# rlvc/FEALESS

Hardware: AMD Instinct MI355X
Metric: frames/sec (640x480 RGB-D x N templates, 20 ICP iters) (higher is better)
Workload: dtype u8

## Files before the change

fealess_amd/_lib.py:

```python
import ctypes as C
import os

_HERE = os.path.dirname(os.path.abspath(__file__))
LIB_PATH = os.environ.get("FEALESS_HIP_LIB") or os.path.join(_HERE, "csrc", "libfealess_hip.so")

FL_OK = 0
FL_ERR_INVALID, FL_ERR_HIP, FL_ERR_ASSERT, FL_ERR_OVERFLOW, FL_ERR_NO_DEVICE, FL_ERR_STATE, FL_ERR_NO_TEMPLATE = -1, -2, -3, -4, -5, -6, -7
FL_MEM_HOST, FL_MEM_DEVICE = 0, 1
FL_ICP_PARITY, FL_ICP_FAST, FL_ICP_POINT_TO_PLANE = 0, 1, 2


class Feature(C.Structure):
    _fields_ = [("x", C.c_int32), ("y", C.c_int32), ("label", C.c_int32)]


class Template(C.Structure):
    _fields_ = [("width", C.c_int32), ("height", C.c_int32), ("offset_x", C.c_int32), ("offset_y", C.c_int32),
                ("pyramid_level", C.c_int32), ("feat_begin", C.c_int32), ("feat_count", C.c_int32)]


class Match(C.Structure):
    _fields_ = [("x", C.c_int32), ("y", C.c_int32), ("similarity", C.c_float), ("class_idx", C.c_int32),
                ("template_id", C.c_int32)]

# ... 133 lines not shown
    "fl_recognize_topk": (_I, [_P, _P, _P, _I, C.POINTER(Intrinsics), C.POINTER(RecognitionParams), _I, _P, C.POINTER(_I)]),
    "fl_recognize_batch_topk": (_I, [_P, _I, C.POINTER(_P), C.POINTER(_P), _I, C.POINTER(Intrinsics), C.POINTER(RecognitionParams), _I, _P,
                                     C.POINTER(_I)]),
    "fl_group_matches": (_I, [_P, _P, _I, _I, C.POINTER(InstanceParams), _P, _P, _P]),
    "fl_recognize_batch_instances": (_I, [_P, _I, C.POINTER(_P), C.POINTER(_P), _I, C.POINTER(Intrinsics), C.POINTER(RecognitionParams),
                                          C.POINTER(InstanceParams), _P, C.POINTER(C.c_int32), C.POINTER(C.c_int32)]),
    "fl_tracker_create": (_I, [_P, _P, _I, _P, _I, _I, _I, _I, _I, _I, C.POINTER(_P)]),
    "fl_tracker_destroy": (None, [_P]),
    "fl_track_batch": (_I, [_P, _I, C.POINTER(_P), _I, _I, _P, _P, C.POINTER(Intrinsics), C.POINTER(TrackParams), _P]),
    "fl_verify_batch": (_I, [_P, _I, C.POINTER(_P), _I, _I, _P, _P, _I, _P, C.POINTER(Intrinsics), C.POINTER(VerifyParams), _P]),
    "fl_nms": (_I, [_P, _I, _F, C.POINTER(_I), C.POINTER(_I)]),
    "fl_export_topk": (_I, [_P, _I, _I, _I, _P]),
    "fl_merge_topk": (_I, [_P, _I, _P, _I]),
    "fl_export_topk_batch": (_I, [_P, _I, _I, _I, _P]),
    "fl_merge_topk_batch": (_I, [_P, _I, _I, _I, _P, _I, C.POINTER(_I)]),
    "fl_refine_matches": (_I, [_P, _I, C.POINTER(C.c_int32), _P, C.POINTER(Intrinsics), C.POINTER(RecognitionParams), _P]),
    "fl_select_best_batch": (_I, [_P, _P, _I, _I, _I, _I, _I, _P]),
    "fl_refine_selected": (_I, [_P, _I, C.POINTER(Intrinsics), C.POINTER(RecognitionParams), _P, C.c_size_t, _P]),
    "fl_last_stage_times": (_I, [_P, C.POINTER(StageTimes)]),
    "fl_frame_counters": (_I, [_P, _I, C.POINTER(C.c_int32)]),
}

DEV_SIGNATURES = {
    "fl_dev_detector_create_host": (_I, [_I, _I, C.POINTER(_I), C.POINTER(_P)]),
    "fl_dev_group_jobs": (_I, [_P, _P, _I, C.POINTER(InstanceParams), _P, _P, _P, _P, _P]),
    "fl_dev_extract_select": (_I, [_P, _I, _P]),
    "fl_dev_front_images": (_I, [_P, _P, _P, _I, _I, _I, _I, _P, C.c_size_t]),
    "fl_dev_tracker_create_host": (_I, [_I, _I, _I, _I, _I, C.POINTER(_P)]),
    "fl_dev_tracker_stage_ms": (_I, [_P, C.POINTER(C.c_float)]),
    "fl_dev_tracker_verify_ms": (_I, [_P, C.POINTER(C.c_float)]),
    "fl_dev_cq_window_addr": (None, [C.c_uint, _I, _I, C.POINTER(C.c_uint), C.POINTER(C.c_uint), C.POINTER(_I)]),
    "fl_dev_cq_window_taps": (None, [_P, C.c_uint, _I, _I, _I, _I, _P]),
    "fl_dev_scan_items": (_I, [_P, _I, _I, _I, C.c_uint, _P, _I, _P, _I, _P]),
}


def dev(lib, name):
    fn = getattr(lib, name)
    fn.restype, fn.argtypes = DEV_SIGNATURES[name]
    return fn


class MgResult(C.Structure):
    _fields_ = [("status", C.c_int32), ("found", C.c_int32), ("best", Match), ("pose", C.c_float * 16)]


FL_MG_ID_BYTES = 128
MG_LIB_PATH = os.path.join(_HERE, "mg", "libfealess_mg.so")
MG_SIGNATURES = {
    "fl_mg_unique_id": (_I, [_P, C.c_size_t]),
    "fl_mg_create": (_I, [_P, _P, _I, _I, _I, _I, _I, C.POINTER(_P)]),
    "fl_mg_destroy": (None, [_P]),
    "fl_mg_last_error": (C.c_char_p, [_P]),
    "fl_mg_recognize_batch": (_I, [_P, _I, C.POINTER(_P), C.POINTER(_P), _I, C.POINTER(Intrinsics), C.POINTER(RecognitionParams), _P]),
    "fl_mg_last_stats": (_I, [_P, C.POINTER(C.c_int32), C.POINTER(C.c_size_t), C.POINTER(C.c_size_t)]),
}

_lib = None
_mg_lib = None


def load_mg():
    global _mg_lib
    if _mg_lib is None:
        load()
        if not os.path.exists(MG_LIB_PATH):
# ... 26 lines not shown
```

fealess_amd/csrc/fl_context.hip:

```cpp
#include "fl_internal.h"
#include <stdlib.h>
#include <stdarg.h>
#include <string.h>
#include <algorithm>

int fl_set_error(fl_context *ctx, int code, const char *fmt, ...)
{
  if (ctx) {
    va_list ap;
    va_start(ap, fmt);
    vsnprintf(ctx->err, sizeof(ctx->err), fmt, ap);
    va_end(ap);
  }
  return code;
}

int fl_scratch(fl_context *ctx, size_t bytes, void **out)
{
  if (int rc = fl_context_join(ctx)) return rc;
  if (bytes > ctx->scratch_bytes) {
    if (ctx->scratch) {
      FL_HIP(ctx, hipStreamSynchronize(ctx->stream));
      FL_HIP(ctx, hipFree(ctx->scratch));
      ctx->scratch = nullptr;
// ... 46 lines not shown
  const long mode = ctx->opt.pipeline_icp;
  if (ctx->icp_stream && ctx->icp_stream_mode != mode) {
    FL_HIP(ctx, hipStreamSynchronize(ctx->icp_stream));
    FL_HIP(ctx, hipStreamDestroy(ctx->icp_stream));
    ctx->icp_stream = nullptr;
  }
  if (!ctx->icp_stream) {
    int least = 0, greatest = 0;
    FL_HIP(ctx, hipDeviceGetStreamPriorityRange(&least, &greatest));
    FL_HIP(ctx, hipStreamCreateWithPriority(&ctx->icp_stream, hipStreamNonBlocking, mode == 2 ? greatest : (mode == 3 ? least : 0)));
    ctx->icp_stream_mode = mode;
  }
  if (!ctx->ev_icp_tail) FL_HIP(ctx, hipEventCreateWithFlags(&ctx->ev_icp_tail, hipEventDisableTiming));
  *out = ctx->icp_stream;
  return FL_OK;
}

extern "C" int fl_abi_version(void) { return FL_ABI_VERSION; }

struct FlOptionName { const char *name, *env; long fl_context::Options::*field; bool hex; long lo, hi; };
static const FlOptionName fl_option_names[] = {
  {"scan_prune", "FL_SCAN_PRUNE", &fl_context::Options::scan_prune, false, 0, 1},
  {"scan_prune_mid", "FL_SCAN_PRUNE_MID", &fl_context::Options::scan_prune_mid, true, -1, 0xFF},
  {"icp_wide", "FL_ICP_WIDE", &fl_context::Options::icp_wide, false, -1, 1},
  {"icp_occ", "FL_ICP_OCC", &fl_context::Options::icp_occ, false, 0, 5},
  {"icp_order", "FL_ICP_ORDER", &fl_context::Options::icp_order, false, 0, 1},
  {"icp_wg_per_cu", "FL_ICP_WG_PER_CU", &fl_context::Options::icp_wg_per_cu, false, 0, 3},
  {"eager_frontend", "FL_EAGER_FRONTEND", &fl_context::Options::eager_frontend, false, 0, 1},
  {"dev_poison", "FL_DEV_POISON", &fl_context::Options::dev_poison, false, 0, 1},
  {"ws_pad", "FL_DEV_WS_PAD", &fl_context::Options::ws_pad, false, 0, 16l << 20},
  {"pipeline_icp", "FL_PIPELINE_ICP", &fl_context::Options::pipeline_icp, false, 0, 3},
  {"frontend_chunk_rows", "FL_FRONTEND_CHUNK_ROWS", &fl_context::Options::frontend_chunk_rows, false, 0, 60 * 1024},
  {"scan_run", "FL_SCAN_RUN", &fl_context::Options::scan_run, false, 0, 64},
};

static bool fl_option_valid(const FlOptionName &o, long v)
{
  if (v < o.lo || v > o.hi) return false;
  if (o.field == &fl_context::Options::frontend_chunk_rows) return v % 60 == 0;
  return o.field != &fl_context::Options::icp_occ || v == 0 || v >= 4;
}

extern "C" int fl_context_create(int device, fl_context **out)
{
  if (!out) return FL_ERR_INVALID;
  *out = nullptr;
  int n = 0;
  if (hipGetDeviceCount(&n) != hipSuccess || n <= 0) return FL_ERR_NO_DEVICE;
  if (device < 0 || device >= n) return FL_ERR_INVALID;
  fl_context *ctx = new fl_context();
  ctx->device = device;
  if (hipSetDevice(device) != hipSuccess ||
      hipStreamCreateWithFlags(&ctx->own_stream, hipStreamNonBlocking) != hipSuccess) {
    delete ctx;
    return FL_ERR_HIP;
  }
  ctx->stream = ctx->own_stream;
  {
    hipDeviceProp_t prop;
    if (hipGetDeviceProperties(&prop, device) == hipSuccess && prop.multiProcessorCount > 0) ctx->cus = prop.multiProcessorCount;
  }
  for (const FlOptionName &o : fl_option_names)
    if (const char *e = getenv(o.env)) {
      const long v = o.hex ? (long)strtoul(e, nullptr, 16) : atol(e);
      if (fl_option_valid(o, v)) ctx->opt.*(o.field) = v;
    }
// ... 65 lines not shown
extern "C" size_t fl_lm_label_stride(int w, int h, int T)
{
  size_t W = (size_t)(w / T), H = (size_t)(h / T);
  size_t pad = W * H + 16 * W + 64;
  size_t s = (size_t)T * T * W * H + pad;
  return (s + 63) & ~(size_t)63;
}

extern "C" int fl_detector_create(fl_context *ctx, int modalities, int levels, const int *T_at_level,
                                  fl_detector **out)
{
  if (!ctx || !out || !T_at_level) return FL_ERR_INVALID;
  if (modalities < 1 || modalities > FL_MAX_MODALITIES || levels < 1 || levels > FL_MAX_LEVELS)
    return fl_set_error(ctx, FL_ERR_INVALID, "modalities must be 1..%d and levels 1..%d", FL_MAX_MODALITIES,
                        FL_MAX_LEVELS);
  for (int l = 0; l < levels; ++l)
    if (T_at_level[l] < 1 || T_at_level[l] > 16) return fl_set_error(ctx, FL_ERR_INVALID, "T out of range");
  fl_detector *det = new fl_detector();
  det->ctx = ctx;
  ++ctx->detectors;
  det->M = modalities;
  det->L = levels;
  for (int l = 0; l < levels; ++l) det->T[l] = T_at_level[l];
  memset(&det->times, 0, sizeof(det->times));
  *out = det;
  return FL_OK;
}

static void free_device_tables(fl_detector *det)
{
  (void)hipFree(det->d_scan_items);
  (void)hipFree(det->d_scan_off);
  (void)hipFree(det->d_fine_hdr);
  (void)hipFree(det->d_fine_feat);
  (void)hipFree(det->d_pyr);
  (void)hipFree(det->d_poses);
  (void)hipFree(det->d_class_first);
  (void)hipFree(det->d_item_enabled);
  (void)hipFree((void *)det->d_depth_ptrs);
  (void)hipFree(det->d_ws);
  (void)hipFree(det->d_results);
  if (det->h_results) (void)hipHostFree(det->h_results);
  det->d_scan_items = nullptr;
  det->n_scan_items = 0;
  det->scan_item_g.clear();
  det->d_scan_off = nullptr;
  det->d_fine_hdr = nullptr;
  det->d_fine_feat = nullptr;
  det->d_pyr = nullptr;
  det->d_poses = nullptr;
  det->d_class_first = nullptr;
  det->d_item_enabled = nullptr;
  det->d_depth_ptrs = nullptr;
  det->d_ws = nullptr;
  det->d_results = nullptr;
  det->h_results = nullptr;
  for (auto &e : det->ev)
    if (e) { (void)hipEventDestroy(e); e = nullptr; }
  for (int b = 0; b < 2; ++b) {
    if (det->ev_done[b]) { (void)hipEventDestroy(det->ev_done[b]); det->ev_done[b] = nullptr; }
    if (det->ev_set_read[b]) { (void)hipEventDestroy(det->ev_set_read[b]); det->ev_set_read[b] = nullptr; }
    det->set_busy[b] = false;
  }
  det->prev_n = 0;
  det->latest_open = false;
  if (det->d_jobs) { (void)hipFree(det->d_jobs); det->d_jobs = nullptr; }
  if (det->d_icp_order) { (void)hipFree(det->d_icp_order); det->d_icp_order = nullptr; }
  det->selected_frames = 0;
  if (det->d_zoom) { (void)hipFree(det->d_zoom); det->d_zoom = nullptr; }
  if (det->d_zoom_src) { (void)hipFree(det->d_zoom_src); det->d_zoom_src = nullptr; det->zoom_src_bytes = 0; }
  for (int b = 0; b < 2; ++b) {
    if (det->d_in[b]) { (void)hipFree(det->d_in[b]); det->d_in[b] = nullptr; }
    if (det->ev_up[b]) { (void)hipEventDestroy(det->ev_up[b]); det->ev_up[b] = nullptr; }
    if (det->ev_read[b]) { (void)hipEventDestroy(det->ev_read[b]); det->ev_read[b] = nullptr; }
    det->read_pending[b] = false;
  }
  if (det->copy_stream) { (void)hipStreamSynchronize(det->copy_stream); (void)hipStreamDestroy(det->copy_stream); det->copy_stream = nullptr; }
}

extern "C" void fl_detector_destroy(fl_detector *det)
// ... 267 lines not shown
  free_device_tables(det);
  det->finalized = false;
  fl_batch_forget(det);
  const int L = det->L, M = det->M;
  int cap = max_candidates > 0 ? max_candidates : (max_candidates < 0 ? -max_candidates : 65536);
  det->cap_hard = max_candidates < 0;
  int cap2 = 1;
  while (cap2 < cap) cap2 <<= 1;
  cap = cap2;

  for (int l = 0; l < L; ++l) {
    FlLevelGeom &g = det->geom[l];
    g.w = w0 >> l;
    g.h = h0 >> l;
    g.T = det->T[l];
    if (g.w <= 0 || g.h <= 0) return fl_set_error(ctx, FL_ERR_INVALID, "level %d is empty", l);
    if (g.w % g.T || g.h % g.T)
      return fl_set_error(ctx, FL_ERR_ASSERT, "level %d: %dx%d not divisible by T=%d (CV_Assert linemod.cpp:1062)", l, g.w,
                          g.h, g.T);
    if ((g.w * g.h) % 16) return fl_set_error(ctx, FL_ERR_ASSERT, "level %d: rows*cols %% 16 != 0 (linemod.cpp:981)", l);
    g.W = g.w / g.T;
    g.H = g.h / g.T;
    g.WH = g.W * g.H;
    size_t s = fl_lm_label_stride(g.w, g.h, g.T);
    if (8 * s > 0xFFFFFFFFull) return fl_set_error(ctx, FL_ERR_INVALID, "linear memory too large");
    g.stride = (uint32_t)s;
    g.zero_off = (uint32_t)(7 * s + (size_t)g.T * g.T * g.WH);
  }

  std::vector<FlScanHdr> scan_hdr;
  std::vector<uint32_t> scan_off;
  std::vector<FlFineHdr> fine_hdr;
  std::vector<FlFineFeat> fine_feat;
  std::vector<FlPyrInfo> pyr;
  std::vector<float> poses;
  std::vector<const uint16_t *> depth_ptrs;
  std::vector<int> class_first;
  int g_idx = 0;
  double scan_bytes = 0.0;
  det->max_tw = det->max_th = 1;
  det->depth_w = det->depth_h = 0;
  for (size_t ci = 0; ci < det->classes.size(); ++ci) {
    FlClass &c = det->classes[ci];
    c.first_g = g_idx;
    class_first.push_back(g_idx);
    if (c.d_depths) {
      if (c.dw != w0 || c.dh != h0)
        return fl_set_error(ctx, FL_ERR_INVALID, "model depth renders must be %dx%d like the frames", w0, h0);
      det->depth_w = c.dw;
      det->depth_h = c.dh;
    }
    for (int p = 0; p < c.n_pyramids; ++p, ++g_idx) {
      const fl_template *tp = &c.templates[(size_t)p * L * M];
      FlPyrInfo pi;
      pi.class_idx = (int)ci;
      pi.template_id = p;
      pi.off_x0 = tp[0].offset_x;
      pi.off_y0 = tp[0].offset_y;
      pi.width0 = tp[0].width;
      pi.height0 = tp[0].height;
      const bool has_depth = c.d_depths && c.has_depth[(size_t)p];
      pi.depth_slot = has_depth ? p : -1;
      pi.pad = 0;
      pyr.push_back(pi);
      det->max_tw = std::max(det->max_tw, std::min(tp[0].width, w0));
      det->max_th = std::max(det->max_th, std::min(tp[0].height, h0));
      for (int k = 0; k < 13; ++k) poses.push_back(c.poses.empty() ? 0.f : c.poses[(size_t)p * 13 + k]);
      depth_ptrs.push_back(has_depth ? c.d_depths + (size_t)p * c.dw * c.dh : nullptr);
      {
        const FlLevelGeom &g = det->geom[L - 1];
        for (int m = 0; m < M; ++m) {
          const fl_template &t = tp[(L - 1) * M + m];
          FlScanHdr h;
          int wf = (t.width - 1) / g.T + 1, hf = (t.height - 1) / g.T + 1;
          int span_x = g.W - wf, span_y = g.H - hf;
          h.P = span_y * g.W + span_x + 1;
          if (h.P > g.WH) h.P = g.WH;
          h.off_begin = (int)scan_off.size();
          h.nf = t.feat_count;
          int n = 0;
          for (int k = 0; k < t.feat_count; ++k) {
            const fl_feature &f = c.features[t.feat_begin + k];
            if (f.x < 0 || f.x >= g.w || f.y < 0 || f.y >= g.h) continue;
            uint32_t off = (uint32_t)f.label * g.stride + (uint32_t)((f.y % g.T) * g.T + (f.x % g.T)) * g.WH +
                           (uint32_t)((f.y / g.T) * g.W + f.x / g.T);
            scan_off.push_back(off);
            ++n;
          }
          while (n % 8) { scan_off.push_back(g.zero_off); ++n; }
          h.n_pad = n;
          scan_hdr.push_back(h);
          const double Pd = h.P > 0 ? (double)h.P : 0.0;
          scan_bytes += (double)t.feat_count * Pd + Pd + (m == 0 ? 2.0 * Pd : 0.0);
        }
      }
      for (int l = 0; l < L - 1; ++l) {
        for (int m = 0; m < M; ++m) {
          const fl_template &t = tp[l * M + m];
          FlFineHdr h;
          h.feat_begin = (int)fine_feat.size();
          h.feat_count = t.feat_count;
          h.width = t.width;
          h.height = t.height;
          for (int k = 0; k < t.feat_count; ++k) {
            const fl_feature &f = c.features[t.feat_begin + k];
            FlFineFeat ff;
            ff.x = (int16_t)f.x;
            ff.y = (int16_t)f.y;
            {
              const int Tl = det->geom[l].T;
              const int rx = ((f.x % Tl) + Tl) % Tl, ry = ((f.y % Tl) + Tl) % Tl;
              ff.gx = (uint8_t)rx;
              ff.gy = (uint8_t)ry;
              ff.qx = (int16_t)((f.x - rx) / Tl);
              ff.qy = (int16_t)((f.y - ry) / Tl);
              ff.label = (uint8_t)f.label;
              ff.pad = 0;
            }
            fine_feat.push_back(ff);
          }
          fine_hdr.push_back(h);
        }
      }
    }
  }
  det->n_pyr = g_idx;
  det->scan_bytes_per_frame = scan_bytes;

  int rc;
  {
    std::vector<FlScanItem> items;
    fl_build_scan_items(scan_hdr, g_idx, M, det->geom[L - 1].WH, det->geom[L - 1].zero_off, scan_off, items);
    det->n_scan_items = (int)items.size();
    det->scan_item_g.clear();
    for (const FlScanItem &it : items) det->scan_item_g.push_back(it.g);
    if ((rc = upload(ctx, items, &det->d_scan_items))) return rc;
  }
  if ((rc = upload(ctx, scan_off, &det->d_scan_off))) return rc;
  if ((rc = upload(ctx, fine_hdr, &det->d_fine_hdr))) return rc;
  if ((rc = upload(ctx, fine_feat, &det->d_fine_feat))) return rc;
  if ((rc = upload(ctx, pyr, &det->d_pyr))) return rc;
  if ((rc = upload(ctx, poses, &det->d_poses))) return rc;
  if ((rc = upload(ctx, class_first, &det->d_class_first))) return rc;
  if ((rc = fl_apply_class_filter(det))) return rc;
  {
    const uint16_t **tmp = nullptr;
    if ((rc = upload(ctx, depth_ptrs, (const uint16_t ***)&tmp))) return rc;
    det->d_depth_ptrs = tmp;
  }

  det->w0 = w0;
  det->h0 = h0;
  det->max_batch = max_batch;
  det->eager_env = ctx->opt.eager_frontend != 0;
  det->poison_env = ctx->opt.dev_poison != 0;
  if ((rc = layout_workspace(det, cap))) return rc;
  if ((rc = fl_icp_prepare(det))) return rc;
  FL_HIP(ctx, hipMalloc((void **)&det->d_results, sizeof(fl_recognition_result) * (size_t)max_batch));
  FL_HIP(ctx, hipHostMalloc((void **)&det->h_results, sizeof(fl_recognition_result) * 2 * (size_t)max_batch,
                            hipHostMallocDefault));
  for (auto &e : det->ev) FL_HIP(ctx, hipEventCreate(&e));
  for (int b = 0; b < 2; ++b) {
    FL_HIP(ctx, hipEventCreateWithFlags(&det->ev_done[b], hipEventDisableTiming));
    FL_HIP(ctx, hipEventCreateWithFlags(&det->ev_set_read[b], hipEventDisableTiming));
  }
  det->finalized = true;
  return FL_OK;
}
```

fealess_amd/csrc/fl_internal.h:

```cpp
#pragma once
#include <hip/hip_runtime.h>
#include <cmath>
#include <stdint.h>
#include <stdio.h>
#include <string>
#include <vector>
#include "../../include/fealess_hip.h"

#define FL_WAVE 64

struct fl_context {
  int device = 0;
  hipStream_t own_stream = nullptr;
  hipStream_t stream = nullptr;
  hipStream_t icp_stream = nullptr;
  long icp_stream_mode = 0;
  hipEvent_t ev_icp_tail = nullptr;
  bool icp_pending = false;
  char err[512] = {0};
  void *scratch = nullptr;
  size_t scratch_bytes = 0;
  void *pinned = nullptr;
  size_t pinned_bytes = 0;
  int cus = 256;
  struct Options {
    long scan_prune = 1;
    long scan_prune_mid = -1;
    long icp_wide = -1;
    long icp_occ = 0;
    long icp_order = 1;
    long icp_wg_per_cu = 0;
    long eager_frontend = 0;
    long dev_poison = 0;
    long ws_pad = 0;
    long pipeline_icp = 3;
    long frontend_chunk_rows = 0;
    long scan_run = 0;
  } opt;
  int detectors = 0;
  bool destroy_pending = false;
};

int fl_set_error(fl_context *ctx, int code, const char *fmt, ...);
int fl_scratch(fl_context *ctx, size_t bytes, void **out);
int fl_pinned(fl_context *ctx, size_t bytes, void **out);
int fl_context_join(fl_context *ctx);
int fl_context_sync_all(fl_context *ctx);
int fl_icp_stream(fl_context *ctx, hipStream_t *out);

#define FL_HIP(ctx, call)                                                                  \
  do {                                                                                     \
    hipError_t e_ = (call);                                                                \
    if (e_ != hipSuccess)                                                                  \
      return fl_set_error((ctx), FL_ERR_HIP, "%s:%d: %s -> %s", __FILE__, __LINE__, #call, \
                          hipGetErrorString(e_));                                          \
  } while (0)

static inline size_t fl_align(size_t v, size_t a) { return (v + a - 1) / a * a; }
static inline bool fl_finite_all(const float *p, size_t n)
{
  for (size_t i = 0; i < n; ++i)
    if (!std::isfinite(p[i])) return false;
  return true;
}

#define FL_MAX_LEVELS 4
#define FL_MAX_MODALITIES 2
#define FL_MAX_FEATURES 63

struct FlScanHdr {
  int32_t P;
  int32_t off_begin;
  int32_t n_pad;
  int32_t nf;
};
struct FlScanItem {
  uint32_t off0[8];
  int32_t g;
  uint32_t chunk_nf;
  struct {
    int32_t P;
    int32_t off_begin;
    uint32_t npad_nf;
  } mod[FL_MAX_MODALITIES];
};
static_assert(sizeof(FlScanItem) == 64 && FL_MAX_MODALITIES == 2, "a dword per lane of a 16-lane load");
#define FL_SCAN_OFF_PAD 8
void fl_build_scan_items(const std::vector<FlScanHdr> &hdr, int n_pyr, int M, int WH, uint32_t zero_off, std::vector<uint32_t> &scan_off,
                         std::vector<FlScanItem> &items);
struct FlFineFeat {
  int16_t x, y;
  int16_t qx, qy;
  uint8_t gx, gy;
  uint8_t label, pad;
};
struct FlFineHdr {
  int32_t feat_begin, feat_count;
  int32_t width, height;
};
struct FlPyrInfo {
  int32_t class_idx, template_id;
  int32_t off_x0, off_y0, width0, height0;
  int32_t depth_slot;
  int32_t pad;
};
struct FlCand {
  int32_t x, y;
  int32_t g;
  float sim;
};

struct FlRefineJob {
  int32_t frame;
  fl_match match;
};

#define FL_TILE 60
#define FL_TILE_WORDS 16
#define FL_TILE_BLOCK_WORDS (66 * FL_TILE_WORDS)
#define FL_NUM_EVENTS 24

struct FlLevelGeom {
  int32_t w, h, T, W, H, WH;
  uint32_t stride;
  uint32_t zero_off;
  size_t quant_off[FL_MAX_MODALITIES];
  size_t lm_off[FL_MAX_MODALITIES];
  size_t spread_off[FL_MAX_MODALITIES];
  size_t bgr_off;
};

struct FlClass {
  std::string id;
  int n_pyramids = 0;
  std::vector<fl_template> templates;
  std::vector<fl_feature> features;
  std::vector<float> poses;
  int first_g = 0;
  uint16_t *d_depths = nullptr;
  std::vector<uint8_t> has_depth;
  int dw = 0, dh = 0;
};

struct FlBatch {
  int n = 0;
  const uint16_t *depth = nullptr;
  size_t depth_stride = 0;
  bool match_only = false;
};

struct fl_detector {
  fl_context *ctx = nullptr;
  int M = 0, L = 0;
  int T[FL_MAX_LEVELS] = {0};
  std::vector<FlClass> classes;
  bool finalized = false;
  int w0 = 0, h0 = 0, max_batch = 0, cap = 0;
  bool cap_hard = false;
  int n_pyr = 0;
  FlLevelGeom geom[FL_MAX_LEVELS];

  FlScanItem *d_scan_items = nullptr;
  int n_scan_items = 0;
  std::vector<int32_t> scan_item_g;
  uint32_t *d_scan_off = nullptr;
  FlFineHdr *d_fine_hdr = nullptr;
  FlFineFeat *d_fine_feat = nullptr;
  FlPyrInfo *d_pyr = nullptr;
  int *d_class_first = nullptr;
  uint8_t *d_item_enabled = nullptr;
  std::vector<std::string> class_filter;
  float *d_poses = nullptr;
  const uint16_t **d_depth_ptrs = nullptr;
  int depth_w = 0, depth_h = 0;
  int max_tw = 0, max_th = 0;

  uint8_t *d_ws = nullptr;
  size_t ws_stride = 0;
  size_t off_bgr = 0, off_depth = 0, off_cand = 0, off_count = 0, off_keys = 0, off_match = 0;
  size_t off_icp = 0, off_tmp = 0;
  size_t off_count_set[2] = {0, 0}, off_match_set[2] = {0, 0};
  int set = 0;
  hipEvent_t ev_set_read[2] = {nullptr, nullptr};
  bool set_busy[2] = {false, false};
  size_t off_tiles = 0;
  bool lazy_capable = false;
  bool lazy = false;
  bool eager_env = false, poison_env = false;
  const uint8_t *lazy_bgr = nullptr;
  hipStream_t copy_stream = nullptr;
  uint8_t *d_in[2] = {nullptr, nullptr};
  hipEvent_t ev_up[2] = {nullptr, nullptr}, ev_read[2] = {nullptr, nullptr};
  bool read_pending[2] = {false, false};
  int in_flip = 0;
  size_t lazy_bgr_stride = 0;
  uint8_t *d_zoom = nullptr;
  uint8_t *d_zoom_src = nullptr;
  size_t zoom_src_bytes = 0;
  int n_pts_max = 0;
// ... 139 lines not shown
```

fealess_amd/csrc/fl_linemod.hip:

```cpp
#include "fl_internal.h"
#include <limits.h>
#include <string.h>

__global__ __launch_bounds__(256) void k_build_lm_generic(const uint8_t *__restrict__ quant, size_t quant_stride,
                                                          uint8_t *__restrict__ lm, size_t lm_stride, int w, int h,
                                                          int T, int W, int WH, uint32_t stride)
{
  const int p = blockIdx.x * 256 + threadIdx.x;
  const int gi = blockIdx.y;
  const uint8_t *q = quant + (size_t)blockIdx.z * quant_stride;
  uint8_t *out = lm + (size_t)blockIdx.z * lm_stride;
  if (p >= WH) return;
  const int gy = gi / T, gx = gi - gy * T;
  const int yt = p / W, xt = p - yt * W;
  const int y = yt * T + gy, x = xt * T + gx;
  unsigned b = 0;
  const int rmax = min(T, h - y), cmax = min(T, w - x);
  for (int r = 0; r < rmax; ++r) {
    const uint8_t *row = q + (size_t)(y + r) * w + x;
    for (int c = 0; c < cmax; ++c) b |= row[c];
  }
  const unsigned bb = b | (b << 8);
#pragma unroll
  for (int ori = 0; ori < 8; ++ori) {
// ... 542 lines not shown
            const unsigned bb = b[u][c] | (b[u][c] << 8);
            const unsigned rot = (bb >> lab[u]) & 0xFFu;
            const unsigned r = (rot & 1u) ? 4u : ((rot & 0x82u) ? 2u : ((rot & 0x44u) ? 1u : 0u));
            packed |= r << (8 * c);
          }
          acc += packed;
        }
      }
      tot0 += acc & 0xFFu;
      tot1 += (acc >> 8) & 0xFFu;
      tot2 += (acc >> 16) & 0xFFu;
      tot3 += acc >> 24;
    }
    const int pos = row * 16 + col4;
    uint32_t key = (tot0 << 8) | (uint32_t)(255 - pos);
    key = max(key, (tot1 << 8) | (uint32_t)(254 - pos));
    key = max(key, (tot2 << 8) | (uint32_t)(253 - pos));
    key = max(key, (tot3 << 8) | (uint32_t)(252 - pos));
#pragma unroll
    for (int s = 32; s >= 1; s >>= 1) key = max(key, (uint32_t)__shfl_xor((int)key, s, 64));
    const int best_score = (int)(key >> 8);
    int best_r = -1, best_c = -1;
    if (best_score > 0) {
      const int bp = 255 - (int)(key & 0xFFu);
      best_r = bp >> 4;
      best_c = bp & 15;
    }
    if (lane == 0) {
      cd.x = (x / T - 8 + best_c) * T + offset;
      cd.y = (y / T - 8 + best_r) * T + offset;
      cd.sim = (best_score * 100.f) / (4 * numFeatures);
      if (cd.sim < a.threshold) cd.g = -1;
      cand[ci] = cd;
    }
  }
}

__global__ __launch_bounds__(256) void k_mark_tiles(RefineArgs a, size_t off_tiles)
{
  __shared__ uint32_t bm[2][FL_TILE_WORDS];
  __shared__ int rlo[2][32 * FL_TILE_WORDS], rhi[2][32 * FL_TILE_WORDS];
  __shared__ int s_all;
  const int wave = threadIdx.x >> 6, lane = threadIdx.x & 63;
  const int frame = blockIdx.x;
  uint8_t *ws = a.ws + (size_t)frame * a.ws_stride;
  for (int i = threadIdx.x; i < 2 * FL_TILE_WORDS; i += 256) bm[0][i] = 0;
  for (int i = threadIdx.x; i < 2 * 32 * FL_TILE_WORDS; i += 256) { rlo[0][i] = 0xFFFF; rhi[0][i] = 0; }
  if (threadIdx.x == 0) s_all = 0;
  __syncthreads();
  const int n = min(*(const int *)(ws + a.off_count), a.cap);
  const FlCand *cand = (const FlCand *)(ws + a.off_cand);
  const int T = a.T, W = a.W, H = a.H;
  const int border = 8 * T;
  const int nstrips = (a.w + FL_TILE - 1) / FL_TILE, nchunks = (a.h + FL_TILE - 1) / FL_TILE;
  for (int ci = wave; ci < n; ci += 4) {
    const FlCand cd = cand[ci];
    const int g = __builtin_amdgcn_readfirstlane(cd.g);
    if (g < 0) continue;
    const FlFineHdr *hdr = a.hdr + ((size_t)g * a.Lm1 + a.level) * a.M;
    const int max_x = a.w - hdr[0].width - border, max_y = a.h - hdr[0].height - border;
    int x = __builtin_amdgcn_readfirstlane(cd.x) * 2 + 1, y = __builtin_amdgcn_readfirstlane(cd.y) * 2 + 1;
    x = max(x, border);
    y = max(y, border);
    x = min(x, max_x);
    y = min(y, max_y);
    const int offset_x = (x / T - 8) * T, offset_y = (y / T - 8) * T;
// ... 153 lines not shown
      m.similarity = __uint_as_float((unsigned)(k.hi >> 32));
      m.template_id = 0x7FFFFFFF - (int)(k.hi & 0xFFFFFFFFu);
      m.class_idx = 0xFFFF - (int)(k.lo >> 32);
      m.y = (0xFFFF - (int)((k.lo >> 16) & 0xFFFF)) - 32768;
      m.x = (0xFFFF - (int)(k.lo & 0xFFFF)) - 32768;
      out[pos] = m;
    }
    __syncthreads();
    if (threadIdx.x == blockDim.x - 1) s_base += s_scan[threadIdx.x];
    __syncthreads();
  }
  if (threadIdx.x == 0) {
    counters[1] = s_base;
    counters[2] = n_raw > a.cap ? 1 : 0;
  }
}

#ifndef FL_SCAN_RUN_AUTO
#define FL_SCAN_RUN_AUTO 8
#endif
#ifndef FL_SCAN_STRIDED
#define FL_SCAN_STRIDED 1
#endif
#define FL_SCAN_FILL 4
static int fl_scan_run(const fl_context *ctx, int items, int n_frames)
{
  if (ctx->opt.scan_run) return (int)ctx->opt.scan_run;
  const long need = (long)FL_SCAN_FILL * ctx->cus * 4 * (ctx->opt.scan_prune ? FL_SCAN_WPE_PRUNED : FL_SCAN_WPE);
  int run = FL_SCAN_RUN_AUTO;
  while (run > 1 && (long)n_frames * ((items + run - 1) / run) < need) run /= 2;
  return run;
}

static int launch_scan_refine_sort(fl_detector *det, int n_frames, float threshold, uint16_t *dbg, int dbg_first,
                                   int dbg_count)
{
  fl_context *ctx = det->ctx;
  const int L = det->L, M = det->M;
  {
    const FlLevelGeom &g = det->geom[L - 1];
    ScanArgs a;
    a.offs = det->d_scan_off;
    a.enabled = det->d_item_enabled;
    a.ws = det->d_ws;
    a.ws_stride = det->ws_stride;
    for (int m = 0; m < FL_MAX_MODALITIES; ++m) a.lm_off[m] = g.lm_off[m < M ? m : 0];
    a.off_count = det->off_count;
    a.off_cand = det->off_cand;
    a.M = M;
    a.W = g.W;
    a.WH = g.WH;
    a.T = g.T;
    a.cap = det->cap;
    a.threshold = threshold;
    a.prune = ctx->opt.scan_prune != 0;
    a.prune_mid = ctx->opt.scan_prune_mid >= 0 ? (unsigned)ctx->opt.scan_prune_mid : FL_SCAN_PRUNE_MID;
    a.dbg = dbg;
    a.dbg_first = dbg_first;
    a.dbg_count = dbg ? dbg_count : 0;
    a.items = det->d_scan_items;
    a.n_items = det->n_scan_items;
    const int items = det->n_scan_items;
    if (items > 0) {
      a.run = fl_scan_run(ctx, items, n_frames);
      const int waves = (items + a.run - 1) / a.run;
      a.bpf = (waves + 3) / 4;
// ... 11 lines not shown
      FL_HIP(ctx, hipGetLastError());
    }
  }
  if (det->have_times) FL_HIP(ctx, hipEventRecord(det->ev[3], ctx->stream));
  for (int l = L - 2; l >= 0; --l) {
    const FlLevelGeom &g = det->geom[l];
    RefineArgs a;
    const bool lazy_level = det->lazy;
    a.hdr = det->d_fine_hdr;
    a.feat = det->d_fine_feat;
    a.ws = det->d_ws;
    a.ws_stride = det->ws_stride;
    for (int m = 0; m < FL_MAX_MODALITIES; ++m) a.spread_off[m] = g.spread_off[m < M ? m : 0];
    a.off_count = det->off_count;
    a.off_cand = det->off_cand;
    a.M = M;
    a.Lm1 = L - 1;
    a.level = l;
    a.w = g.w;
    a.h = g.h;
    a.T = g.T;
    a.W = g.W;
    a.H = g.H;
    a.cap = det->cap;
    a.threshold = threshold;
    if (lazy_level) {
      if (det->have_times) FL_HIP(ctx, hipEventRecord(det->ev[8 + 2 * l], ctx->stream));
      hipLaunchKernelGGL(k_mark_tiles, dim3(n_frames), dim3(256), 0, ctx->stream, a, det->off_tiles);
      FL_HIP(ctx, hipGetLastError());
      int rc = fl_launch_lazy_level(det, n_frames, l);
      if (rc) return rc;
      if (det->have_times) FL_HIP(ctx, hipEventRecord(det->ev[9 + 2 * l], ctx->stream));
    }
    dim3 grid(n_frames >= 64 ? 4 : (n_frames >= 8 ? 32 : 256), n_frames);
    hipLaunchKernelGGL(k_refine, grid, dim3(256), 0, ctx->stream, a);
    FL_HIP(ctx, hipGetLastError());
  }
  if (det->have_times) FL_HIP(ctx, hipEventRecord(det->ev[4], ctx->stream));
  {
    SortArgs a;
    a.pyr = det->d_pyr;
    a.ws = det->d_ws;
    a.ws_stride = det->ws_stride;
    a.off_count = det->off_count;
    a.off_cand = det->off_cand;
    a.off_keys = det->off_keys;
    a.off_match = det->off_match;
    a.cap = det->cap;
    hipLaunchKernelGGL(k_sort_unique, dim3(n_frames), dim3(1024), 0, ctx->stream, a);
    FL_HIP(ctx, hipGetLastError());
  }
  if (det->have_times) FL_HIP(ctx, hipEventRecord(det->ev[5], ctx->stream));
  return FL_OK;
}

int fl_launch_match_core(fl_detector *det, int n_frames, float threshold)
{
  fl_context *ctx = det->ctx;
  if (det->set_busy[det->set]) {
    det->set_busy[det->set] = false;
    FL_HIP(ctx, hipStreamWaitEvent(ctx->stream, det->ev_set_read[det->set], 0));
  }
  FL_HIP(ctx, hipMemset2DAsync(det->d_ws + det->off_count, det->ws_stride, 0, 16, n_frames, ctx->stream));
  for (int l = 0; l < det->L; ++l) {
    const FlLevelGeom &g = det->geom[l];
    for (int m = 0; m < det->M; ++m) {
      if (det->lazy && l < det->L - 1) continue;
      int rc = l == det->L - 1
// ... 724 lines not shown
```

Before: 84310.

## Stage spread windows in LDS for batched candidate refinement

```diff
diff --git a/fealess_amd/_lib.py b/fealess_amd/_lib.py
--- a/fealess_amd/_lib.py
+++ b/fealess_amd/_lib.py
@@ -189,6 +189,10 @@
     "fl_dev_cq_window_addr": (None, [C.c_uint, _I, _I, C.POINTER(C.c_uint), C.POINTER(C.c_uint), C.POINTER(_I)]),
     "fl_dev_cq_window_taps": (None, [_P, C.c_uint, _I, _I, _I, _I, _P]),
     "fl_dev_scan_items": (_I, [_P, _I, _I, _I, C.c_uint, _P, _I, _P, _I, _P]),
+    "fl_dev_refine_pitch": (_I, [_I, _I]),
+    "fl_dev_refine_plan": (_I, [_P, _I, _I, C.c_long, _I, _P]),
+    "fl_dev_refine_kernel": (_I, [_P, _I]),
+    "fl_dev_refine_window_max": (C.c_long, [_P, _I]),
 }
 
 
diff --git a/fealess_amd/csrc/fl_context.hip b/fealess_amd/csrc/fl_context.hip
--- a/fealess_amd/csrc/fl_context.hip
+++ b/fealess_amd/csrc/fl_context.hip
@@ -102,6 +102,8 @@
   {"pipeline_icp", "FL_PIPELINE_ICP", &fl_context::Options::pipeline_icp, false, 0, 3},
   {"frontend_chunk_rows", "FL_FRONTEND_CHUNK_ROWS", &fl_context::Options::frontend_chunk_rows, false, 0, 60 * 1024},
   {"scan_run", "FL_SCAN_RUN", &fl_context::Options::scan_run, false, 0, 64},
+  {"refine_lds", "FL_REFINE_LDS", &fl_context::Options::refine_lds, false, 0, 2},
+  {"refine_lds_bytes", "FL_REFINE_LDS_BYTES", &fl_context::Options::refine_lds_bytes, false, 0, FL_REFINE_LDS_BYTES},
 };
 
 static bool fl_option_valid(const FlOptionName &o, long v)
@@ -233,6 +235,7 @@
   (void)hipFree(det->d_scan_items);
   (void)hipFree(det->d_scan_off);
   (void)hipFree(det->d_fine_hdr);
+  (void)hipFree(det->d_fine_box);
   (void)hipFree(det->d_fine_feat);
   (void)hipFree(det->d_pyr);
   (void)hipFree(det->d_poses);
@@ -247,6 +250,7 @@
   det->scan_item_g.clear();
   det->d_scan_off = nullptr;
   det->d_fine_hdr = nullptr;
+  det->d_fine_box = nullptr;
   det->d_fine_feat = nullptr;
   det->d_pyr = nullptr;
   det->d_poses = nullptr;
@@ -580,6 +584,8 @@
   std::vector<uint32_t> scan_off;
   std::vector<FlFineHdr> fine_hdr;
   std::vector<FlFineFeat> fine_feat;
+  std::vector<FlFineBox> fine_box;
+  for (int l = 0; l < FL_MAX_LEVELS; ++l) det->refine_window_max[l] = 0;
   std::vector<FlPyrInfo> pyr;
   std::vector<float> poses;
   std::vector<const uint16_t *> depth_ptrs;
@@ -643,8 +649,10 @@
         }
       }
       for (int l = 0; l < L - 1; ++l) {
+        FlRect all = {0, 0, -1, -1};
         for (int m = 0; m < M; ++m) {
           const fl_template &t = tp[l * M + m];
+          FlRect box = {0, 0, -1, -1};
           FlFineHdr h;
           h.feat_begin = (int)fine_feat.size();
           h.feat_count = t.feat_count;
@@ -666,8 +674,19 @@
               ff.pad = 0;
             }
             fine_feat.push_back(ff);
+            const FlRect one = {ff.x, ff.y, ff.x, ff.y};
+            box = fl_rect_union(box, one);
           }
           fine_hdr.push_back(h);
+          fine_box.push_back(FlFineBox{(int16_t)box.x0, (int16_t)box.y0, (int16_t)box.x1, (int16_t)box.y1});
+          all = fl_rect_union(all, box);
+        }
+        if (all.x1 >= all.x0) {
+          const FlLevelGeom &gl = det->geom[l];
+          const int ww = std::min(all.x1 - all.x0 + 15 * gl.T + 1 + 3, (gl.w + 3) & ~3);
+          const int hh = std::min(all.y1 - all.y0 + 15 * gl.T + 1, gl.h);
+          const long bytes = (long)fl_refine_pitch(ww, fl_refine_qmask(gl.T)) * hh;
+          det->refine_window_max[l] = std::max(det->refine_window_max[l], bytes);
         }
       }
     }
@@ -687,6 +706,7 @@
   if ((rc = upload(ctx, scan_off, &det->d_scan_off))) return rc;
   if ((rc = upload(ctx, fine_hdr, &det->d_fine_hdr))) return rc;
   if ((rc = upload(ctx, fine_feat, &det->d_fine_feat))) return rc;
+  if ((rc = upload(ctx, fine_box, &det->d_fine_box))) return rc;
   if ((rc = upload(ctx, pyr, &det->d_pyr))) return rc;
   if ((rc = upload(ctx, poses, &det->d_poses))) return rc;
   if ((rc = upload(ctx, class_first, &det->d_class_first))) return rc;
diff --git a/fealess_amd/csrc/fl_internal.h b/fealess_amd/csrc/fl_internal.h
--- a/fealess_amd/csrc/fl_internal.h
+++ b/fealess_amd/csrc/fl_internal.h
@@ -36,6 +36,8 @@
     long pipeline_icp = 3;
     long frontend_chunk_rows = 0;
     long scan_run = 0;
+    long refine_lds = 0;
+    long refine_lds_bytes = 0;
   } opt;
   int detectors = 0;
   bool destroy_pending = false;
@@ -98,6 +100,9 @@
   int32_t feat_begin, feat_count;
   int32_t width, height;
 };
+struct FlFineBox {
+  int16_t x0, y0, x1, y1;
+};
 struct FlPyrInfo {
   int32_t class_idx, template_id;
   int32_t off_x0, off_y0, width0, height0;
@@ -114,6 +119,69 @@
   int32_t frame;
   fl_match match;
 };
+
+#define FL_REFINE_LDS_BYTES 65536
+#define FL_REFINE_GROUP_MAX 8
+#define FL_REFINE_BLOCK 256
+struct FlRect { int x0, y0, x1, y1; };
+__host__ __device__ inline int fl_refine_pitch(int width, uint32_t qmask)
+{
+  int q = (width + 3) >> 2;
+  while (!((qmask >> (q & 31)) & 1u)) ++q;
+  return q * 4;
+}
+__host__ __device__ inline uint32_t fl_refine_qmask(int T)
+{
+  uint32_t mask = 0;
+  int best = 33;
+  for (int q = 0; q < 32; q += 4) {
+    int n[32] = {0}, worst = 0;
+    for (int row = 0; row < 8; ++row)
+      for (int cg = 0; cg < 4; ++cg) {
+        const int b = (T * (row * q + cg)) & 31;
+        if (++n[b] > worst) worst = n[b];
+      }
+    if (worst < best) { best = worst; mask = 0; }
+    if (worst == best) mask |= 1u << q;
+  }
+  return mask;
+}
+__host__ __device__ inline FlRect fl_rect_union(FlRect a, FlRect b)
+{
+  if (a.x1 < a.x0) return b;
+  if (b.x1 < b.x0) return a;
+  FlRect r;
+  r.x0 = a.x0 < b.x0 ? a.x0 : b.x0;
+  r.y0 = a.y0 < b.y0 ? a.y0 : b.y0;
+  r.x1 = a.x1 > b.x1 ? a.x1 : b.x1;
+  r.y1 = a.y1 > b.y1 ? a.y1 : b.y1;
+  return r;
+}
+__host__ __device__ inline long fl_refine_window_bytes(FlRect r, uint32_t qmask)
+{
+  if (r.x1 < r.x0) return 0;
+  return (long)fl_refine_pitch(r.x1 - (r.x0 & ~3) + 1, qmask) * (r.y1 - r.y0 + 1);
+}
+template <typename C>
+__host__ __device__ inline int fl_refine_plan(const C *rects, int n, int max_len, long budget, uint32_t qmask, FlRect *uni)
+{
+  FlRect u = {rects[0], rects[1], rects[2], rects[3]};
+  int len = 1;
+  while (len < n && len < max_len) {
+    const C *c = rects + 4 * len;
+    const FlRect r = {c[0], c[1], c[2], c[3]};
+    const FlRect v = fl_rect_union(u, r);
+    if (fl_refine_window_bytes(v, qmask) > budget) break;
+    u = v;
+    ++len;
+  }
+  *uni = u;
+  return len;
+}
+extern "C" int fl_dev_refine_pitch(int width, int T);
+extern "C" int fl_dev_refine_plan(const int32_t *rects, int n, int max_len, long budget, int T, int32_t *uni);
+extern "C" int fl_dev_refine_kernel(const fl_detector *det, int level);
+extern "C" long fl_dev_refine_window_max(const fl_detector *det, int level);
 
 #define FL_TILE 60
 #define FL_TILE_WORDS 16
@@ -165,6 +233,9 @@
   std::vector<int32_t> scan_item_g;
   uint32_t *d_scan_off = nullptr;
   FlFineHdr *d_fine_hdr = nullptr;
+  FlFineBox *d_fine_box = nullptr;
+  long refine_window_max[FL_MAX_LEVELS] = {0};
+  int refine_ran[FL_MAX_LEVELS] = {0};
   FlFineFeat *d_fine_feat = nullptr;
   FlPyrInfo *d_pyr = nullptr;
   int *d_class_first = nullptr;
diff --git a/fealess_amd/csrc/fl_linemod.hip b/fealess_amd/csrc/fl_linemod.hip
--- a/fealess_amd/csrc/fl_linemod.hip
+++ b/fealess_amd/csrc/fl_linemod.hip
@@ -598,6 +598,259 @@
       cd.sim = (best_score * 100.f) / (4 * numFeatures);
       if (cd.sim < a.threshold) cd.g = -1;
       cand[ci] = cd;
+    }
+  }
+}
+
+static_assert(FL_MAX_MODALITIES == 2, "the first modality's packed sums wait in LDS while the second is staged");
+static_assert(FL_REFINE_LDS_BYTES + 4 * 64 * FL_REFINE_GROUP_MAX + 10 * FL_REFINE_BLOCK + 64 <= 70 * 1024, "LDS beside three ICP workgroups");
+
+__device__ __noinline__ uint4 refine_stage_tail(const uint8_t *p, const uint8_t *end)
+{
+  uint32_t v[4] = {0, 0, 0, 0};
+  for (int i = 0; i < 16; ++i)
+    if (p + i < end) v[i >> 2] |= (uint32_t)p[i] << (8 * (i & 3));
+  return make_uint4(v[0], v[1], v[2], v[3]);
+}
+
+__device__ __forceinline__ uint32_t refine_resp4(uint32_t p, int lab)
+{
+  const uint32_t M = 0x01010101u;
+  const uint32_t lo = (0xFFu >> lab) * M;
+  const uint32_t rot = ((p >> lab) & lo) | ((p << (8 - lab)) & ~lo);
+  const uint32_t t1 = rot & M;
+  const uint32_t t2 = ((rot >> 1) | (rot >> 7)) & M;
+  const uint32_t t3 = ((rot >> 2) | (rot >> 6)) & M;
+  const uint32_t n1 = t1 ^ M, n2 = t2 ^ M;
+  return (t1 << 2) | (((t2 << 1) | (t3 & n2)) & ((n1 << 1) | n1));
+}
+
+#ifdef FL_REFINE_STATS
+__device__ unsigned long long d_refine_stats[4];
+#endif
+
+template <int TT>
+__attribute__((amdgpu_num_vgpr(128)))
+__global__ __launch_bounds__(256) void k_refine_lds(RefineArgs a, const FlFineBox *box, int budget, uint32_t qmask)
+{
+  __shared__ __attribute__((aligned(16))) uint8_t s_win[FL_REFINE_LDS_BYTES];
+  __shared__ uint32_t s_keyacc[64 * FL_REFINE_GROUP_MAX > FL_REFINE_BLOCK ? 64 * FL_REFINE_GROUP_MAX : FL_REFINE_BLOCK];
+  __shared__ int16_t s_rect[4 * FL_REFINE_BLOCK];
+  __shared__ uint16_t s_idx[FL_REFINE_BLOCK];
+  __shared__ int s_plan[5];
+  const int tid = threadIdx.x, wave = tid >> 6, lane = tid & 63;
+  uint8_t *ws = a.ws + (size_t)blockIdx.x * a.ws_stride;
+  const int n = min(*(const int *)(ws + a.off_count), a.cap);
+  FlCand *cand = (FlCand *)(ws + a.off_cand);
+  const int row = lane >> 2, col4 = (lane & 3) * 4;
+  const int T = TT ? TT : a.T, W = a.W, H = a.H;
+  const int border = 8 * T, offset = T / 2 + (T % 2 - 1);
+  for (int blk = 0; blk < n; blk += FL_REFINE_BLOCK) {
+    const int nb = min(FL_REFINE_BLOCK, n - blk);
+    uint32_t key = 0xFFFFFFFFu;
+    FlRect rc = {0, 0, -1, -1};
+    if (tid < nb) {
+      const FlCand cd = cand[blk + tid];
+      if (cd.g >= 0) {
+        const size_t hi = ((size_t)cd.g * a.Lm1 + a.level) * a.M;
+        int x = cd.x * 2 + 1, y = cd.y * 2 + 1;
+        x = max(x, border);
+        y = max(y, border);
+        x = min(x, a.w - a.hdr[hi].width - border);
+        y = min(y, a.h - a.hdr[hi].height - border);
+        const int offset_x = (x / T - 8) * T, offset_y = (y / T - 8) * T;
+        FlRect b = {0, 0, -1, -1};
+        for (int m = 0; m < a.M; ++m) {
+          const FlFineBox fb = box[hi + m];
+          const FlRect one = {fb.x0, fb.y0, fb.x1, fb.y1};
+          b = fl_rect_union(b, one);
+        }
+        if (b.x1 >= b.x0) {
+          rc.x0 = max(0, b.x0 + offset_x);
+          rc.y0 = max(0, b.y0 + offset_y);
+          rc.x1 = min(a.w - 1, b.x1 + offset_x + 15 * T);
+          rc.y1 = min(a.h - 1, b.y1 + offset_y + 15 * T);
+          if (rc.x1 < rc.x0 || rc.y1 < rc.y0) rc = FlRect{0, 0, -1, -1};
+        }
+        key = ((uint32_t)((x / T + 0x4000) & 0x7FFF) << 16) | (uint32_t)((y / T + 0x4000) & 0x7FFF);
+      }
+    }
+    s_keyacc[tid] = key;
+    __syncthreads();
+    if (tid < nb) {
+      int rank = 0;
+      for (int u = 0; u < nb; ++u) {
+        const uint32_t k = s_keyacc[u];
+        rank += (k < key || (k == key && u < tid)) ? 1 : 0;
+      }
+      s_idx[rank] = (uint16_t)tid;
+      s_rect[4 * rank + 0] = (int16_t)rc.x0;
+      s_rect[4 * rank + 1] = (int16_t)rc.y0;
+      s_rect[4 * rank + 2] = (int16_t)rc.x1;
+      s_rect[4 * rank + 3] = (int16_t)rc.y1;
+    }
+    const int nvalid = __syncthreads_count(key != 0xFFFFFFFFu);
+    for (int gs = 0; gs < nvalid;) {
+      if (tid == 0) {
+        FlRect u;
+        s_plan[0] = fl_refine_plan(s_rect + 4 * gs, nvalid - gs, FL_REFINE_GROUP_MAX, (long)budget, qmask, &u);
+        s_plan[1] = u.x0 & ~3;
+        s_plan[2] = u.y0;
+        s_plan[3] = u.x1;
+        s_plan[4] = u.y1;
+      }
+      __syncthreads();
+      const int len = s_plan[0], ux0 = s_plan[1], uy0 = s_plan[2], ux1 = s_plan[3], uy1 = s_plan[4];
+      const bool have = ux1 >= ux0;
+      const int pitch = have ? fl_refine_pitch(ux1 - ux0 + 1, qmask) : 16;
+      const int lane_lds = row * T * pitch + col4 * T;
+#ifdef FL_REFINE_STATS
+      if (tid == 0) {
+        if (blk == 0 && gs == 0) atomicAdd(&d_refine_stats[0], 1ull);
+        atomicAdd(&d_refine_stats[1], 1ull);
+        atomicAdd(&d_refine_stats[2], have ? (unsigned long long)a.M * pitch * (uy1 - uy0 + 1) : 0ull);
+        atomicAdd(&d_refine_stats[3], (unsigned long long)len);
+      }
+#endif
+      for (int m = 0; m < a.M; ++m) {
+        const uint8_t *sp = ws + a.spread_off[m];
+        if (have) {
+          const int cpr = pitch >> 4, total = (uy1 - uy0 + 1) * cpr;
+          const uint8_t *end = sp + (size_t)a.w * a.h;
+          for (int c0 = tid; c0 < total; c0 += 4 * 256) {
+            uint4 v[4];
+#pragma unroll
+            for (int u = 0; u < 4; ++u) {
+              const int c = c0 + u * 256;
+              if (c < total) {
+                const int r = c / cpr, j = c - r * cpr;
+                const uint8_t *p = sp + (size_t)(uy0 + r) * a.w + (size_t)(ux0 + 16 * j);
+                v[u] = p + 16 <= end ? ld16(p) : refine_stage_tail(p, end);
+              }
+            }
+#pragma unroll
+            for (int u = 0; u < 4; ++u) {
+              const int c = c0 + u * 256;
+              if (c < total) *(uint4 *)(s_win + 16 * (size_t)c) = v[u];
+            }
+          }
+        }
+        __syncthreads();
+        for (int j = wave; j < len; j += 4) {
+          const int ci = blk + s_idx[gs + j];
+          FlCand cd = cand[ci];
+          const int g = __builtin_amdgcn_readfirstlane(cd.g);
+          const FlFineHdr *hdr = a.hdr + ((size_t)g * a.Lm1 + a.level) * a.M;
+          const int max_x = a.w - hdr[0].width - border;
+          const int max_y = a.h - hdr[0].height - border;
+          int x = __builtin_amdgcn_readfirstlane(cd.x) * 2 + 1, y = __builtin_amdgcn_readfirstlane(cd.y) * 2 + 1;
+          x = max(x, border);
+          y = max(y, border);
+          x = min(x, max_x);
+          y = min(y, max_y);
+          const int offset_x = (x / T - 8) * T, offset_y = (y / T - 8) * T;
+          const int offx_t = offset_x / T, offy_t = offset_y / T;
+          const FlFineHdr h = hdr[m];
+          const FlFineFeat *ff = a.feat + h.feat_begin;
+          const int feat_count = __builtin_amdgcn_readfirstlane(h.feat_count);
+          uint32_t acc = 0;
+          int f_xy = 0, f_q = 0, f_g = 0;
+          if (lane < feat_count) {
+            const FlFineFeat f = ff[lane];
+            f_xy = (int)(uint16_t)f.x | ((int)(uint16_t)f.y << 16);
+            f_q = (int)(uint16_t)f.qx | ((int)(uint16_t)f.qy << 16);
+            f_g = (int)f.gx | ((int)f.gy << 8) | ((int)f.label << 16);
+          }
+          const FlFineBox fb = box[((size_t)g * a.Lm1 + a.level) * a.M + m];
+          const bool usual = fb.x0 + offset_x >= 0 && fb.y0 + offset_y >= 0 && fb.x1 + offset_x + 16 * T <= a.w &&
+                             fb.y1 + offset_y + 16 * T <= a.h && feat_count <= 64 && __all(((f_g >> 16) & 0xFF) < 8);
+          if (__builtin_amdgcn_readfirstlane((int)usual)) {
+            const int f_off = ((f_xy >> 16) + offset_y - uy0) * pitch + ((int)(int16_t)(f_xy & 0xFFFF) + offset_x - ux0);
+            for (int k = 0; k < feat_count; k += 8) {
+              uint32_t b[8][4];
+#pragma unroll
+              for (int u = 0; u < 8; ++u) {
+                const uint8_t *p0 = s_win + __builtin_amdgcn_readlane(f_off, min(k + u, feat_count - 1)) + lane_lds;
+#pragma unroll
+                for (int c = 0; c < 4; ++c) b[u][c] = p0[c * T];
+              }
+#pragma unroll
+              for (int u = 0; u < 8; ++u) {
+                const int lab = (__builtin_amdgcn_readlane(f_g, min(k + u, feat_count - 1)) >> 16) & 0xFF;
+                const uint32_t r = refine_resp4(b[u][0] | (b[u][1] << 8) | (b[u][2] << 16) | (b[u][3] << 24), lab);
+                acc += k + u < feat_count ? r : 0u;
+              }
+            }
+          } else
+          for (int k = 0; k < feat_count; k += 8) {
+            uint32_t b[8][4];
+            int lab[8];
+#pragma unroll
+            for (int u = 0; u < 8; ++u) {
+              const int idx = min(k + u, feat_count - 1);
+              const int xy = __builtin_amdgcn_readlane(f_xy, idx), qq = __builtin_amdgcn_readlane(f_q, idx), gl = __builtin_amdgcn_readlane(f_g, idx);
+              const int fx = (int)(int16_t)(xy & 0xFFFF) + offset_x, fy = (int)(int16_t)(xy >> 16) + offset_y;
+              const bool in = (k + u < feat_count) && fx >= 0 && fy >= 0 && fx < a.w && fy < a.h;
+              lab[u] = (gl >> 16) & 0xFF;
+              const int gx = gl & 0xFF, gy = (gl >> 8) & 0xFF;
+              const int lm_x = (int)(int16_t)(qq & 0xFFFF) + offx_t, lm_y = (int)(int16_t)(qq >> 16) + offy_t;
+              if (in && lm_x + 15 < W && lm_y + 15 < H) {
+                const uint8_t *p0 = s_win + ((fy - uy0) * pitch + (fx - ux0)) + lane_lds;
+#pragma unroll
+                for (int c = 0; c < 4; ++c) b[u][c] = p0[c * T];
+              } else {
+                uint32_t r4 = refine_slow_path(sp, in, lm_x + col4, lm_y + row, gx, gy, T, W, H, a.w);
+#pragma unroll
+                for (int c = 0; c < 4; ++c) b[u][c] = (r4 >> (8 * c)) & 0xFFu;
+              }
+            }
+#pragma unroll
+            for (int u = 0; u < 8; ++u) {
+              uint32_t packed = 0;
+#pragma unroll
+              for (int c = 0; c < 4; ++c) {
+                const unsigned bb = b[u][c] | (b[u][c] << 8);
+                const unsigned rot = (bb >> lab[u]) & 0xFFu;
+                const unsigned r = (rot & 1u) ? 4u : ((rot & 0x82u) ? 2u : ((rot & 0x44u) ? 1u : 0u));
+                packed |= r << (8 * c);
+              }
+              acc += packed;
+            }
+          }
+          if (m + 1 < a.M) {
+            s_keyacc[j * 64 + lane] = acc;
+            continue;
+          }
+          const uint32_t acc0 = a.M > 1 ? s_keyacc[j * 64 + lane] : 0u;
+          const uint32_t tot0 = (acc0 & 0xFFu) + (acc & 0xFFu), tot1 = ((acc0 >> 8) & 0xFFu) + ((acc >> 8) & 0xFFu);
+          const uint32_t tot2 = ((acc0 >> 16) & 0xFFu) + ((acc >> 16) & 0xFFu), tot3 = (acc0 >> 24) + (acc >> 24);
+          int numFeatures = 0;
+          for (int mm = 0; mm < a.M; ++mm) numFeatures += hdr[mm].feat_count;
+          const int pos = row * 16 + col4;
+          uint32_t best = (tot0 << 8) | (uint32_t)(255 - pos);
+          best = max(best, (tot1 << 8) | (uint32_t)(254 - pos));
+          best = max(best, (tot2 << 8) | (uint32_t)(253 - pos));
+          best = max(best, (tot3 << 8) | (uint32_t)(252 - pos));
+#pragma unroll
+          for (int s = 32; s >= 1; s >>= 1) best = max(best, (uint32_t)__shfl_xor((int)best, s, 64));
+          const int best_score = (int)(best >> 8);
+          int best_r = -1, best_c = -1;
+          if (best_score > 0) {
+            const int bp = 255 - (int)(best & 0xFFu);
+            best_r = bp >> 4;
+            best_c = bp & 15;
+          }
+          if (lane == 0) {
+            cd.x = (x / T - 8 + best_c) * T + offset;
+            cd.y = (y / T - 8 + best_r) * T + offset;
+            cd.sim = (best_score * 100.f) / (4 * numFeatures);
+            if (cd.sim < a.threshold) cd.g = -1;
+            cand[ci] = cd;
+          }
+        }
+        __syncthreads();
+      }
+      gs += len;
     }
   }
 }
@@ -817,6 +1070,34 @@
   return run;
 }
 
+#ifndef FL_REFINE_LDS_FRAMES_PER_CU
+#define FL_REFINE_LDS_FRAMES_PER_CU 1
+#endif
+static bool fl_refine_use_lds(const fl_detector *det, int level, int n_frames, long *budget)
+{
+  const fl_context *ctx = det->ctx;
+  *budget = ctx->opt.refine_lds_bytes ? ctx->opt.refine_lds_bytes : (long)FL_REFINE_LDS_BYTES;
+  if (ctx->opt.refine_lds == 1 || det->refine_window_max[level] > *budget) return false;
+  return ctx->opt.refine_lds == 2 || n_frames >= FL_REFINE_LDS_FRAMES_PER_CU * ctx->cus;
+}
+
+extern "C" int fl_dev_refine_pitch(int width, int T) { return fl_refine_pitch(width, fl_refine_qmask(T)); }
+extern "C" int fl_dev_refine_plan(const int32_t *rects, int n, int max_len, long budget, int T, int32_t *uni)
+{
+  FlRect u;
+  const int len = fl_refine_plan(rects, n, max_len, budget, fl_refine_qmask(T), &u);
+  if (uni) { uni[0] = u.x0; uni[1] = u.y0; uni[2] = u.x1; uni[3] = u.y1; }
+  return len;
+}
+extern "C" int fl_dev_refine_kernel(const fl_detector *det, int level)
+{
+  return det && level >= 0 && level < det->L - 1 ? det->refine_ran[level] : -1;
+}
+extern "C" long fl_dev_refine_window_max(const fl_detector *det, int level)
+{
+  return det && level >= 0 && level < det->L - 1 ? det->refine_window_max[level] : -1;
+}
+
 static int launch_scan_refine_sort(fl_detector *det, int n_frames, float threshold, uint16_t *dbg, int dbg_first,
                                    int dbg_count)
 {
@@ -894,8 +1175,33 @@
       if (rc) return rc;
       if (det->have_times) FL_HIP(ctx, hipEventRecord(det->ev[9 + 2 * l], ctx->stream));
     }
-    dim3 grid(n_frames >= 64 ? 4 : (n_frames >= 8 ? 32 : 256), n_frames);
-    hipLaunchKernelGGL(k_refine, grid, dim3(256), 0, ctx->stream, a);
+    long budget;
+    if (fl_refine_use_lds(det, l, n_frames, &budget)) {
+      const uint32_t qmask = fl_refine_qmask(g.T);
+      const dim3 grid(n_frames), block(256);
+      switch (g.T) {
+      case 4: hipLaunchKernelGGL(k_refine_lds<4>, grid, block, 0, ctx->stream, a, det->d_fine_box, (int)budget, qmask); break;
+      case 5: hipLaunchKernelGGL(k_refine_lds<5>, grid, block, 0, ctx->stream, a, det->d_fine_box, (int)budget, qmask); break;
+      case 8: hipLaunchKernelGGL(k_refine_lds<8>, grid, block, 0, ctx->stream, a, det->d_fine_box, (int)budget, qmask); break;
+      default: hipLaunchKernelGGL(k_refine_lds<0>, grid, block, 0, ctx->stream, a, det->d_fine_box, (int)budget, qmask); break;
+      }
+      det->refine_ran[l] = 2;
+#ifdef FL_REFINE_STATS
+      {
+        unsigned long long st[4], zero[4] = {0, 0, 0, 0};
+        FL_HIP(ctx, hipStreamSynchronize(ctx->stream));
+        FL_HIP(ctx, hipMemcpyFromSymbol(st, HIP_SYMBOL(d_refine_stats), sizeof(st)));
+        FL_HIP(ctx, hipMemcpyToSymbol(HIP_SYMBOL(d_refine_stats), zero, sizeof(zero)));
+        fprintf(stderr, "k_refine_lds level %d: %d frames, %llu with candidates, %.2f groups per such frame, %.0f bytes staged per group, "
+                "%.2f candidates per group\n", l, n_frames, st[0], st[0] ? (double)st[1] / st[0] : 0.0, st[1] ? (double)st[2] / st[1] : 0.0,
+                st[1] ? (double)st[3] / st[1] : 0.0);
+      }
+#endif
+    } else {
+      dim3 grid(n_frames >= 64 ? 4 : (n_frames >= 8 ? 32 : 256), n_frames);
+      hipLaunchKernelGGL(k_refine, grid, dim3(256), 0, ctx->stream, a);
+      det->refine_ran[l] = 1;
+    }
     FL_HIP(ctx, hipGetLastError());
   }
   if (det->have_times) FL_HIP(ctx, hipEventRecord(det->ev[4], ctx->stream));
```

Measured after the change: 87530 (median of 6 runs). 1.04x the previous value.
